# psipred/merizo_search

Hardware: AMD Instinct MI355X
Metric: queries/sec, exact 128-d cosine top-10 (recall@10 vs brute force = 1.0000) (higher is better)
Workload: dtype f32

## Files before the change

merizo_search_amd/csrc/ms_scan_pf16.h:

```cpp
#pragma once
#include "ms_scan_pf.h"

typedef _Float16 f16x8 __attribute__((ext_vector_type(8)));
constexpr uint32_t MS_PF16_MAGIC = 0x3631464du;
#define MS_PF_ERR_F16X2 5.5e-4f
#define MS_PF_ERR_F16X1 1.05e-3f

template <int KL, int NW, bool SAMPLE, bool MASK, int NQP>
__global__ __launch_bounds__(64 * NW, NW / 4) void ms_scan_pf16_kernel(const ScanParams p) {
    static_assert(NQP == 1 || NQP == 2, "query parts");
    static_assert(NW == 4 || NW == 8, "one or two waves per SIMD");
    constexpr int PPW = 16 / NW;
#ifdef MS_STAMP
    const unsigned long long tl_entry = __builtin_amdgcn_s_memrealtime();
    unsigned long long tl_setup = 0, tl_first = 0, tl_loop = 0;
#endif
    if (ms_gate_closed(p.gate, p.gate_epoch)) return;
    extern __shared__ __attribute__((aligned(16))) char smem[];
    typedef __attribute__((address_space(3))) char lds_char_t;
    typedef volatile __attribute__((address_space(3))) uint32_t lds_flag_t;
    typedef __attribute__((address_space(3))) ms_u32x2 lds_cand_t;
    const int tid = threadIdx.x, lane = tid & 63;
    const int wave = __builtin_amdgcn_readfirstlane(tid >> 6);
    const int r = lane & 31, h = lane >> 5;
    lds_flag_t *arrived = (lds_flag_t *)((lds_char_t *)smem + PF2_OFF_CNT);
    const float *auxring = reinterpret_cast<const float *>(smem + PF2_OFF_AUX);

    const int bid = blockIdx.x;
    const int per_super = 8 * p.n_qgroups;
    const int super = bid / per_super, within = bid % per_super;
    const int stream = super * 8 + (within & 7);
    const int qg = within >> 3;
    if (stream >= p.n_streams) return;
    const int64_t row_begin = (int64_t)stream * p.rows_per_stream;
    const int64_t row_end = (row_begin + p.rows_per_stream < p.n) ? row_begin + p.rows_per_stream : p.n;
    const int nfull = (int)((row_end - row_begin) >> 6);
    const int rem = (int)((row_end - row_begin) & 63);
    const int ntl = SAMPLE ? (nfull < p.max_tiles ? nfull : p.max_tiles) : nfull + (rem > 0 ? 1 : 0);
    constexpr bool mask_on = MASK;

    const int qtile = qg * NW + wave;
    const bool has_q = qtile < p.n_qtiles;
    if (tid < PF2_ARR) arrived[tid] = 0u;
    __syncthreads();
    const uint32_t ring_lds = __builtin_amdgcn_readfirstlane((uint32_t)(uintptr_t)(lds_char_t *)smem);

    const uint32_t voff = (uint32_t)(16 * lane);
    const uint64_t img0 = (uint64_t)(uintptr_t)p.pf_image + (uint64_t)(row_begin >> 6) * 16384u + (uint32_t)(1024 * PPW) * (uint32_t)wave;
    uint64_t it_sb = 0;
    uint32_t it_dst = 0;
    auto issue_prep = [&](int t) __attribute__((always_inline)) {
        const uint64_t b = img0 + (uint64_t)t * 16384u;
        const uint32_t b_lo = (uint32_t)__builtin_amdgcn_readfirstlane((uint32_t)b);
        const uint32_t b_hi = (uint32_t)__builtin_amdgcn_readfirstlane((uint32_t)(b >> 32));
        it_sb = ((uint64_t)b_hi << 32) | (uint64_t)b_lo;
        it_dst = (uint32_t)__builtin_amdgcn_readfirstlane(ring_lds + (uint32_t)(t % PF2_R) * 16384u + (uint32_t)(1024 * PPW) * (uint32_t)wave);
    };
    auto issue_piece = [&](auto i_c) __attribute__((always_inline)) {
        constexpr int I = decltype(i_c)::value;
        if constexpr (I < PPW) {
            const uint32_t d = (uint32_t)__builtin_amdgcn_readfirstlane(it_dst);
            const uint32_t lo = (uint32_t)__builtin_amdgcn_readfirstlane((uint32_t)it_sb), hi = (uint32_t)__builtin_amdgcn_readfirstlane((uint32_t)(it_sb >> 32));
            ms_glds_s16<1024 * I>(d + 1024 * I, voff, ((uint64_t)hi << 32) | (uint64_t)lo);
        }
    };
    auto issue_aux = [&](int t) __attribute__((always_inline)) {
        if constexpr (MASK) {
            int64_t row = row_begin + (int64_t)t * 64 + lane;
            if (row >= p.n) row = p.n - 1;
            const uint32_t dst = wave == 0 ? ring_lds + PF2_OFF_AUX + (uint32_t)(t % PF2_AUXR) * 256u
                                           : ring_lds + PF2_OFF_DUMMY + (uint32_t)(wave - 1) * 256u;
            ms_glds_v4((uint32_t)__builtin_amdgcn_readfirstlane(dst), p.lengths + row);
        }
    };
    auto issue_tile = [&](int t) __attribute__((always_inline)) {
        issue_prep(t);
        issue_piece(std::integral_constant<int, 0>{}); issue_piece(std::integral_constant<int, 1>{});
        issue_piece(std::integral_constant<int, 2>{}); issue_piece(std::integral_constant<int, 3>{});
        issue_aux(t);
    };
    auto wait_own = [&](auto n_c) __attribute__((always_inline)) {
        constexpr int N = decltype(n_c)::value;
        ms_pf2_vmcnt<(PPW + (MASK ? 1 : 0)) * N>();
    };
    const uint32_t arr_lds = ring_lds + PF2_OFF_CNT;
    auto publish = [&](int t) __attribute__((always_inline)) {
        const uint32_t a_ = arr_lds + 4u * (uint32_t)(t & (PF2_ARR - 1));
        uint32_t pub_a, pub_one;
        asm volatile("v_mov_b32 %0, %2\n\tv_mov_b32 %1, 1\n\ts_mov_b64 exec, 1\n\tds_add_u32 %0, %1\n\ts_mov_b64 exec, -1"
                     : "=&v"(pub_a), "=&v"(pub_one) : "s"(a_) : "memory");
    };
    uint32_t seen = 0;
    auto read_arrived = [&](int t) __attribute__((always_inline)) { seen = arrived[t & (PF2_ARR - 1)]; };
    auto wait_arrived = [&](int t) __attribute__((always_inline)) {
        const uint32_t need = (uint32_t)NW * (uint32_t)(t / PF2_ARR + 1);
        uint32_t sv_, spins_, av_;
        static_assert(PF2_ARR == 16, "the mask below");
        asm volatile("s_waitcnt lgkmcnt(0)\n\t"
                     "v_readfirstlane_b32 %0, %2\n\t"
                     "s_cmp_ge_u32 %0, %5\n\t"
                     "s_setprio 2\n\t"
                     "s_cbranch_scc1 2f\n\t"
                     "s_setprio 0\n\t"
                     "s_and_b32 %0, %4, 15\n\t"
                     "s_lshl_b32 %0, %0, 2\n\t"
                     "s_add_u32 %0, %0, %6\n\t"
                     "v_mov_b32 %3, %0\n\t"
                     "s_mov_b32 %1, 0\n\t"
                     "1:\n\t"
                     "s_sleep 1\n\t"
                     "ds_read_b32 %2, %3\n\t"
                     "s_add_u32 %1, %1, 1\n\t"
                     "s_waitcnt lgkmcnt(0)\n\t"
                     "v_readfirstlane_b32 %0, %2\n\t"
                     "s_cmp_ge_u32 %0, %5\n\t"
                     "s_cbranch_scc1 2f\n\t"
                     "s_cmp_lt_u32 %1, 0x1000000\n\t"
                     "s_cbranch_scc1 1b\n\t"
                     "s_trap 2\n\t"
                     "2:"
                     : "=&s"(sv_), "=&s"(spins_), "+v"(seen), "=&v"(av_) : "s"(t), "s"(need), "s"(arr_lds) : "memory", "scc");
        asm volatile("" ::: "memory");
    };
    const int qidx = qtile * 32 + r;
    const bool q_valid = qidx < p.nq;
    const bool hist_on = !SAMPLE && p.hist != nullptr && p.lb_s != nullptr;
    f32x4 qv[16];
    float pre_lb = -INFINITY, pre_stp = 0.0f, pre_qlen = 0.0f;
    uint32_t pre_magic = MS_PF16_MAGIC, pre_n = (uint32_t)p.n;
    int pre_sr = 0;
    if (has_q) {
        const uint32_t *trailer = reinterpret_cast<const uint32_t *>(reinterpret_cast<const char *>(p.pf_image) + (size_t)((p.n + 63) >> 6) * 16384u);
        pre_magic = trailer[0];
        pre_sr = (int)trailer[1];
        pre_n = trailer[2];
        const f32x4 *src = reinterpret_cast<const f32x4 *>(p.qn + (size_t)(q_valid ? qidx : 0) * MS_DIM + 64 * h);
#pragma unroll
        for (int i = 0; i < 16; ++i) qv[i] = src[i];
        if (!SAMPLE && p.lb_s != nullptr) pre_lb = p.lb_s[qidx];
        if (hist_on && q_valid) pre_stp = p.hstep[qidx];
        if (MASK && p.qlen != nullptr && q_valid) pre_qlen = p.qlen[qidx];
    }
    asm volatile("" ::: "memory");
#pragma unroll
    for (int t = 0; t < PF2_D; ++t)
        if (t < ntl) issue_tile(t);

    if (!has_q) {
        if (ntl > 0) {
            if (ntl >= PF2_D) wait_own(std::integral_constant<int, PF2_D - PF2_W>{}); else ms_pf2_vmcnt<0>();
#pragma unroll
            for (int t = 0; t < PF2_W; ++t)
                if (t < ntl) publish(t);
        }
        for (int t = 0; t < ntl; ++t) {
            if (t + 1 < ntl) { read_arrived(t + 1); wait_arrived(t + 1); }
            if (t + PF2_D < ntl) {
                issue_tile(t + PF2_D);
                wait_own(std::integral_constant<int, PF2_D - PF2_W>{});
            } else {
                ms_pf2_vmcnt<0>();
            }
            if (t + PF2_W < ntl) publish(t + PF2_W);
        }
        return;
    }

    ScanState<SAMPLE ? 1 : KL> st;
    ScanHist hg;
    f16x8 qh[8], ql[NQP == 2 ? 8 : 1];
#pragma unroll
    for (int j = 0; j < (SAMPLE ? 1 : KL); ++j) { st.ls[j] = -INFINITY; st.li[j] = MS_IDX_NONE; }
    st.floor = -INFINITY;
    st.tau = -INFINITY;
    if (!SAMPLE && p.lb_s != nullptr) {
        const float lb = pre_lb;
        st.floor = (lb == -INFINITY) ? -INFINITY : nextafterf(lb, -INFINITY);
        st.tau = st.floor;
    }
    if (!q_valid) { st.floor = INFINITY; st.tau = INFINITY; }
    if (!SAMPLE && (p.debug_flags & 1)) { st.floor = INFINITY; st.tau = INFINITY; }
    hg.counters = nullptr; hg.base = 0.0f; hg.step = 0.0f; hg.inv_step = 0.0f;
    if (hist_on && q_valid) {
        const float stp = pre_stp, lb = pre_lb;
        if (stp > 0.0f && lb > -INFINITY) { hg.counters = p.hist + (size_t)qidx * 16; hg.base = lb; hg.step = stp; hg.inv_step = 1.0f / stp; }
    }
    float up = 1.0f, down = 1.0f;
    {
        const uint32_t magic = (uint32_t)__builtin_amdgcn_readfirstlane((int)pre_magic);
        const int sr = __builtin_amdgcn_readfirstlane(pre_sr);
        const uint32_t img_n = (uint32_t)__builtin_amdgcn_readfirstlane((int)pre_n);
        if (magic != MS_PF16_MAGIC || img_n != (uint32_t)p.n) __builtin_trap();
        f32x4 v[16];
        float m = 0.0f;
        float rinv = 1.0f;
        if (p.qraw_eps > 0.0f) {
            float ss = 0.0f;
#pragma unroll
            for (int i = 0; i < 16; ++i) { ss += qv[i].x * qv[i].x; ss += qv[i].y * qv[i].y; ss += qv[i].z * qv[i].z; ss += qv[i].w * qv[i].w; }
            ss = ss + ms_xor32_f(ss, h);
            rinv = 1.0f / fmaxf(sqrtf(ss), p.qraw_eps);
        }
#pragma unroll
        for (int i = 0; i < 16; ++i) {
            v[i] = q_valid ? qv[i] * rinv : f32x4{0.0f, 0.0f, 0.0f, 0.0f};
            m = fmaxf(m, fmaxf(fmaxf(fabsf(v[i].x), fabsf(v[i].y)), fmaxf(fabsf(v[i].z), fabsf(v[i].w))));
        }
        m = fmaxf(m, ms_xor32_f(m, h));
        int sq = 0;
        if (m > 0.0f && m < INFINITY) sq = 13 - ((int)((__float_as_uint(m) >> 23) & 0xFFu) - 127);
        sq = sq > 60 ? 60 : (sq < -60 ? -60 : sq);
        const float qs = __uint_as_float((uint32_t)(127 + sq) << 23);
        up = __uint_as_float((uint32_t)(127 + sr + sq) << 23);
        down = __uint_as_float((uint32_t)(127 - sr - sq) << 23);
#pragma unroll
        for (int b = 0; b < 8; ++b) {
            const f32x4 a0 = v[2 * b] * qs, a1 = v[2 * b + 1] * qs;
            const float x[8] = {a0.x, a0.y, a0.z, a0.w, a1.x, a1.y, a1.z, a1.w};
#pragma unroll
            for (int j = 0; j < 8; ++j) {
                const float c = fminf(fmaxf(x[j], -65504.0f), 65504.0f);
                const _Float16 hi16 = (_Float16)c;
                qh[b][j] = hi16;
                if constexpr (NQP == 2) ql[b][j] = (_Float16)(c - (float)hi16);
            }
        }
    }
    float tau_s = st.tau * up;
    const float my_qlen = (mask_on && p.qlen != nullptr && q_valid) ? pre_qlen : 0.0f;
    const float qlen_eff = mask_on ? my_qlen : INFINITY;
    const float mincov_eff = mask_on ? p.mincov : 0.0f;
    float smax = -INFINITY;
    auto apply_mask = [&](f32x16 &acc, int t, int half) __attribute__((always_inline)) {
        const f32x4 *ax = reinterpret_cast<const f32x4 *>(auxring + (t & (PF2_AUXR - 1)) * 64 + 32 * half + 4 * h);
#pragma unroll
        for (int g = 0; g < 4; ++g) {
            const f32x4 len4 = ax[2 * g];
#pragma unroll
            for (int j = 0; j < 4; ++j) {
                const float mk = (qlen_eff >= len4[j] * mincov_eff) ? 1.0f : 0.0f;
                acc[4 * g + j] = acc[4 * g + j] * mk;
            }
        }
    };
    bool neg_tau = !SAMPLE && mask_on && (__ballot(st.tau < 0.0f) != 0);
    const bool pace_on = !SAMPLE && p.prog != nullptr;
    constexpr int PACE_LEAD = 48;
    int pace_left = 16384;
    auto pace = [&](int t) __attribute__((always_inline)) {
        if (wave != 0 || (t & 15) != 0) return;
        const uint64_t line = (uint64_t)(uintptr_t)(p.prog + (size_t)stream * 16);
        const uint32_t l_lo = (uint32_t)__builtin_amdgcn_readfirstlane((uint32_t)line), l_hi = (uint32_t)__builtin_amdgcn_readfirstlane((uint32_t)(line >> 32));
        const uint64_t sline = ((uint64_t)l_hi << 32) | (uint64_t)l_lo;
        const uint32_t tag = p.prog_epoch << 24;
        if (lane == 0) __hip_atomic_store(p.prog + (size_t)stream * 16 + qg, tag | (uint32_t)t, __ATOMIC_RELAXED, __HIP_MEMORY_SCOPE_AGENT);
        if (t < PACE_LEAD) return;
        typedef uint32_t u32x16_ __attribute__((ext_vector_type(16)));
        for (; pace_left > 0; --pace_left) {
            u32x16_ w;
            asm volatile("s_load_dwordx16 %0, %1, 0x0 glc\n\ts_waitcnt lgkmcnt(0)" : "=s"(w) : "s"(sline) : "memory");
            uint32_t mn = 0xFFFFFFu;
#pragma unroll
            for (int i = 0; i < 16; ++i) {
                const uint32_t v = ((w[i] >> 24) == p.prog_epoch) ? (w[i] & 0xFFFFFFu) : 0u;
                if (i < p.n_qgroups) mn = v < mn ? v : mn;
            }
            if ((uint32_t)t <= mn + (uint32_t)PACE_LEAD) break;
            __builtin_amdgcn_s_sleep(64);
        }
    };
    auto retau = [&]() __attribute__((always_inline)) { tau_s = st.tau * up; };

    uint32_t ccnt = 0;
    auto cand_slot = [&](uint32_t c) __attribute__((always_inline)) -> lds_cand_t * {
        return (lds_cand_t *)((lds_char_t *)smem + PF2_OFF_CAND + (wave * PF2_CAND) * 512) + c * 64 + lane;
    };
    auto flush = [&]() __attribute__((always_inline)) {
        for (uint32_t c = 0; __ballot(ccnt > c) != 0; ++c) {
            const ms_u32x2 e = *cand_slot(c < PF2_CAND ? c : 0);
            const float v = (ccnt > c) ? __uint_as_float(e.x) : -INFINITY;
            ms_lane_insert<SAMPLE ? 1 : KL>(st, v, e.y, 0, h);
            ms_lane_insert<SAMPLE ? 1 : KL>(st, v, e.y, 1, h);
        }
        ccnt = 0;
        retau();
    };
    constexpr bool VISIT2 = !(MASK && (NQP == 2 || KL >= 16));
    auto visit_v2 = [&](f32x16 &sc_v, int t, int half, bool check_rows) __attribute__((always_inline)) {
        if (mask_on) apply_mask(sc_v, t, half);
        const uint32_t sub_row0 = (uint32_t)(row_begin + (int64_t)t * 64) + (uint32_t)(32 * half + 4 * h);
#pragma unroll 1
        for (;;) {
            bool ovf = false;
            float g0, g1, g2, g3;
            asm("v_max3_f32 %0, %4, %5, %6\n\tv_max3_f32 %1, %8, %9, %10\n\tv_max3_f32 %2, %12, %13, %14\n\tv_max3_f32 %3, %16, %17, %18\n\t"
                "v_max_f32 %0, %0, %7\n\tv_max_f32 %1, %1, %11\n\tv_max_f32 %2, %2, %15\n\tv_max_f32 %3, %3, %19"
                : "=&v"(g0), "=&v"(g1), "=&v"(g2), "=&v"(g3)
                : "v"(sc_v[0]), "v"(sc_v[1]), "v"(sc_v[2]), "v"(sc_v[3]), "v"(sc_v[4]), "v"(sc_v[5]), "v"(sc_v[6]), "v"(sc_v[7]), "v"(sc_v[8]),
                  "v"(sc_v[9]), "v"(sc_v[10]), "v"(sc_v[11]), "v"(sc_v[12]), "v"(sc_v[13]), "v"(sc_v[14]), "v"(sc_v[15]));
#define MS_PF16_REG(I)                                                                                                   \
            {                                                                                                            \
                const float ss = sc_v[I];                                                                                \
                const uint32_t row = sub_row0 + (uint32_t)(8 * ((I) >> 2) + ((I) & 3));                                    \
                bool pass = ss > tau_s;                                                                                  \
                if (check_rows) pass = pass && ((int64_t)row < row_end);                                                 \
                if (pass) {                                                                                              \
                    if (ccnt < (uint32_t)PF2_CAND) {                                                                     \
                        const float s_ = ss * down;                       \
                        if (hg.counters != nullptr) ms_hist_count(hg, s_);                                               \
                        *cand_slot(ccnt) = ms_u32x2{__float_as_uint(s_), row};                                           \
                        ccnt += 1;                                                                                       \
                        sc_v[I] = -INFINITY;                                                                             \
                    } else {                                                                                             \
                        ovf = true;                                                                                      \
                    }                                                                                                    \
                }                                                                                                        \
            }
#define MS_PF16_GROUP(G, GM) if (__ballot(GM > tau_s) != 0) { MS_PF16_REG(4 * (G)) MS_PF16_REG(4 * (G) + 1) MS_PF16_REG(4 * (G) + 2) MS_PF16_REG(4 * (G) + 3) }
            MS_PF16_GROUP(0, g0) MS_PF16_GROUP(1, g1) MS_PF16_GROUP(2, g2) MS_PF16_GROUP(3, g3)
#undef MS_PF16_GROUP
#undef MS_PF16_REG
            if (__builtin_expect(__ballot(ovf) == 0, 1)) break;
            flush();
        }
    };
    auto visit_v1 = [&](f32x16 &sc_v, int t, int half, bool check_rows) __attribute__((always_inline)) {
        if (mask_on) apply_mask(sc_v, t, half);
        const uint32_t sub_row0 = (uint32_t)(row_begin + (int64_t)t * 64) + (uint32_t)(32 * half + 4 * h);
        uint32_t regs = 0;
        {
            float g0, g1, g2, g3;
            asm("v_max3_f32 %0, %4, %5, %6\n\tv_max3_f32 %1, %8, %9, %10\n\tv_max3_f32 %2, %12, %13, %14\n\tv_max3_f32 %3, %16, %17, %18\n\t"
                "v_max_f32 %0, %0, %7\n\tv_max_f32 %1, %1, %11\n\tv_max_f32 %2, %2, %15\n\tv_max_f32 %3, %3, %19"
                : "=&v"(g0), "=&v"(g1), "=&v"(g2), "=&v"(g3)
                : "v"(sc_v[0]), "v"(sc_v[1]), "v"(sc_v[2]), "v"(sc_v[3]), "v"(sc_v[4]), "v"(sc_v[5]), "v"(sc_v[6]), "v"(sc_v[7]), "v"(sc_v[8]),
                  "v"(sc_v[9]), "v"(sc_v[10]), "v"(sc_v[11]), "v"(sc_v[12]), "v"(sc_v[13]), "v"(sc_v[14]), "v"(sc_v[15]));
#define MS_PF16_GROUP(G, GM)                                                                                             \
            if (__ballot(GM > tau_s) != 0) {                                                                             \
                _Pragma("unroll") for (int j = 0; j < 4; ++j) regs |= (__ballot(sc_v[4 * (G) + j] > tau_s) != 0 ? 1u : 0u) << (4 * (G) + j); \
            }
            MS_PF16_GROUP(0, g0) MS_PF16_GROUP(1, g1) MS_PF16_GROUP(2, g2) MS_PF16_GROUP(3, g3)
#undef MS_PF16_GROUP
        }
#pragma unroll 1
        while (regs != 0u) {
            const int i = __builtin_ctz(regs);
            regs &= regs - 1u;
            const uint64_t m0_ = (i & 1) ? ~0ull : 0ull, m1_ = (i & 2) ? ~0ull : 0ull, m2_ = (i & 4) ? ~0ull : 0ull, m3_ = (i & 8) ? ~0ull : 0ull;
            float l1[8], l2[4], l3[2], ss;
#define MS_SEL(D, A, B, M) asm("v_cndmask_b32 %0, %1, %2, %3" : "=v"(D) : "v"(A), "v"(B), "s"(M))
#pragma unroll
            for (int j = 0; j < 8; ++j) MS_SEL(l1[j], sc_v[2 * j], sc_v[2 * j + 1], m0_);
#pragma unroll
            for (int j = 0; j < 4; ++j) MS_SEL(l2[j], l1[2 * j], l1[2 * j + 1], m1_);
            MS_SEL(l3[0], l2[0], l2[1], m2_); MS_SEL(l3[1], l2[2], l2[3], m2_);
            MS_SEL(ss, l3[0], l3[1], m3_);
#undef MS_SEL
            const uint32_t row = sub_row0 + (uint32_t)(8 * (i >> 2) + (i & 3));
            const float s = ss * down;
            bool pass = ss > tau_s;
            if (check_rows) pass = pass && ((int64_t)row < row_end);
            if (pass) {
                if (hg.counters != nullptr) ms_hist_count(hg, s);
                *cand_slot(ccnt) = ms_u32x2{__float_as_uint(s), row};
                ccnt += 1;
            }
            if (__builtin_expect(__ballot(ccnt >= PF2_CAND) != 0, 0)) flush();
        }
    };
    auto visit = [&](f32x16 &sc_v, int t, int half, bool check_rows) __attribute__((always_inline)) {
        if constexpr (VISIT2) visit_v2(sc_v, t, half, check_rows); else visit_v1(sc_v, t, half, check_rows);
    };

#ifdef MS_STAMP
    unsigned long long sp_t0 = 0, sp_sync = 0, sp_vis = 0, sp_nvis = 0, sp_chain = 0, sp_hist = 0, sp_lgkm = 0, sp_flow = 0;
#define PF2_T0() sp_t0 = __builtin_amdgcn_s_memtime()
#define PF2_ACC(V) { const unsigned long long now_ = __builtin_amdgcn_s_memtime(); V += now_ - sp_t0; sp_t0 = now_; }
#else
#define PF2_T0()
#define PF2_ACC(V)
#endif
    f32x4 fr[16];
    f32x16 acc0, acc1;
#pragma unroll
    for (int i = 0; i < 16; ++i) { acc0[i] = -INFINITY; acc1[i] = -INFINITY; }

    auto frag_base = [&](int t) __attribute__((always_inline)) -> const f32x4 * {
        return reinterpret_cast<const f32x4 *>(smem + (size_t)(t % PF2_R) * 16384 + 16 * lane);
    };
    auto filter = [&](int t, f32x16 &pv0, f32x16 &pv1) __attribute__((always_inline)) {
        if (SAMPLE) {
            if (mask_on && t > 0) { apply_mask(pv0, t - 1, 0); apply_mask(pv1, t - 1, 1); }
#pragma unroll
            for (int i = 0; i < 16; ++i) { smax = (pv0[i] > smax) ? pv0[i] : smax; smax = (pv1[i] > smax) ? pv1[i] : smax; }
        } else {
            float mx, mx1;
#define MS_PF16_MAX(M, PV)                                                                                                                        \
            asm("v_max3_f32 %0, %1, %2, %3\n\tv_max3_f32 %0, %0, %4, %5\n\tv_max3_f32 %0, %0, %6, %7\n\tv_max3_f32 %0, %0, %8, %9\n\t"             \
                "v_max3_f32 %0, %0, %10, %11\n\tv_max3_f32 %0, %0, %12, %13\n\tv_max3_f32 %0, %0, %14, %15\n\tv_max_f32 %0, %0, %16"               \
                : "=&v"(M) : "v"(PV[0]), "v"(PV[1]), "v"(PV[2]), "v"(PV[3]), "v"(PV[4]), "v"(PV[5]), "v"(PV[6]), "v"(PV[7]), "v"(PV[8]), "v"(PV[9]), \
                  "v"(PV[10]), "v"(PV[11]), "v"(PV[12]), "v"(PV[13]), "v"(PV[14]), "v"(PV[15]))
            MS_PF16_MAX(mx, pv0);
            MS_PF16_MAX(mx1, pv1);
#undef MS_PF16_MAX
            const bool hit0 = __ballot(mx > tau_s) != 0, hit1 = __ballot(mx1 > tau_s) != 0;
            if (__builtin_expect(hit0 || hit1 || neg_tau, 0)) {
                PF2_T0();
                if (t > 0) {
                    if (hit0 || neg_tau) visit(pv0, t - 1, 0, false);
                    if (hit1 || neg_tau) visit(pv1, t - 1, 1, false);
                }
                if (mask_on) neg_tau = __ballot(st.tau < 0.0f) != 0;
#ifdef MS_STAMP
                sp_nvis += 1;
#endif
                PF2_ACC(sp_vis)
            }
        }
    };
    auto stage = [&](auto steady_c, int t, f32x16 &out0, f32x16 &out1) __attribute__((always_inline)) {
        constexpr bool STEADY = decltype(steady_c)::value;
        PF2_T0();
        asm volatile("s_waitcnt lgkmcnt(0)" ::: "memory");
        PF2_ACC(sp_lgkm)
        if (STEADY || t + 1 < ntl) wait_arrived(t + 1);
        PF2_ACC(sp_sync)
        filter(t, out0, out1);
#pragma unroll
        for (int i = 0; i < 16; ++i) { out0[i] = 0.0f; out1[i] = 0.0f; }
        const f32x4 *src = frag_base(t + 1);
        const bool issuing = STEADY || t + PF2_D < ntl;
#define MS_PF2_BLOCK(B)                                                                                               \
        {                                                                                                             \
            const f16x8 f0 = __builtin_bit_cast(f16x8, fr[2 * (B)]), f1 = __builtin_bit_cast(f16x8, fr[2 * (B) + 1]);   \
            out0 = __builtin_amdgcn_mfma_f32_32x32x16_f16(f0, qh[B], out0, 0, 0, 0);                                  \
            out1 = __builtin_amdgcn_mfma_f32_32x32x16_f16(f1, qh[B], out1, 0, 0, 0);                                  \
            if constexpr (NQP == 2) {                                                                                 \
                out0 = __builtin_amdgcn_mfma_f32_32x32x16_f16(f0, ql[B], out0, 0, 0, 0);                              \
                out1 = __builtin_amdgcn_mfma_f32_32x32x16_f16(f1, ql[B], out1, 0, 0, 0);                              \
            }                                                                                                         \
            __builtin_amdgcn_sched_barrier(0);                                                                        \
            fr[2 * (B)] = src[64 * (2 * (B))];                                                                        \
            fr[2 * (B) + 1] = src[64 * (2 * (B) + 1)];                                                                \
        }
        MS_PF2_BLOCK(0)
        __builtin_amdgcn_sched_barrier(0);
        MS_PF2_BLOCK(1)
        if (STEADY || issuing) issue_prep(t + PF2_D);
        __builtin_amdgcn_sched_barrier(0);
        MS_PF2_BLOCK(2)
        if (STEADY || issuing) issue_piece(std::integral_constant<int, 0>{});
        __builtin_amdgcn_sched_barrier(0);
        MS_PF2_BLOCK(3)
        if (STEADY || issuing) issue_piece(std::integral_constant<int, 1>{});
        __builtin_amdgcn_sched_barrier(0);
        MS_PF2_BLOCK(4)
        if (STEADY || issuing) issue_piece(std::integral_constant<int, 2>{});
        __builtin_amdgcn_sched_barrier(0);
        MS_PF2_BLOCK(5)
        if (STEADY || issuing) { issue_piece(std::integral_constant<int, 3>{}); issue_aux(t + PF2_D); }
        __builtin_amdgcn_sched_barrier(0);
        MS_PF2_BLOCK(6)
        PF2_ACC(sp_chain)
        if (STEADY || issuing) wait_own(std::integral_constant<int, PF2_D - PF2_W>{}); else ms_pf2_vmcnt<0>();
        PF2_ACC(sp_flow)
        if (STEADY || t + PF2_W < ntl) publish(t + PF2_W);
        read_arrived(t + 2);
        __builtin_amdgcn_sched_barrier(0);
        MS_PF2_BLOCK(7)
#undef MS_PF2_BLOCK
#ifdef MS_STAMP
        asm volatile("s_nop 0" : "+v"(out0), "+v"(out1));
#endif
        PF2_ACC(sp_chain)
    };

#ifdef MS_STAMP
    const unsigned long long sp_c0 = __builtin_amdgcn_s_memtime(), sp_r0 = __builtin_amdgcn_s_memrealtime();
    tl_setup = sp_r0;
#endif
    if (ntl > 0) {
        if (ntl >= PF2_D) wait_own(std::integral_constant<int, PF2_D - PF2_W>{}); else ms_pf2_vmcnt<0>();
#pragma unroll
        for (int t = 0; t < PF2_W; ++t)
            if (t < ntl) publish(t);
        read_arrived(0);
        wait_arrived(0);
#ifdef MS_STAMP
        tl_first = __builtin_amdgcn_s_memrealtime();
#endif
        {
            const f32x4 *src = frag_base(0);
#pragma unroll
            for (int f = 0; f < 16; ++f) fr[f] = src[64 * f];
        }
        read_arrived(1);
        const int fetch_phase = 2 * wave, read_phase = (2 * wave + 2) & (HIST_PERIOD - 1);
        const int hist_area = wave & 3;
        auto hist_step = [&](int t) __attribute__((always_inline)) {
            const int phase = t & (HIST_PERIOD - 1);
            if (phase == fetch_phase) {
                const uint64_t hb = (uint64_t)(uintptr_t)p.hist + (uint64_t)qtile * 2048u;
                const uint32_t hb_lo = (uint32_t)__builtin_amdgcn_readfirstlane((uint32_t)hb);
                const uint32_t hb_hi = (uint32_t)__builtin_amdgcn_readfirstlane((uint32_t)(hb >> 32));
                const uint64_t shb = ((uint64_t)hb_hi << 32) | (uint64_t)hb_lo;
                const uint32_t dst = (uint32_t)__builtin_amdgcn_readfirstlane(ring_lds + PF2_OFF_HIST + (uint32_t)hist_area * 2048u);
                ms_glds_s16_sc1<0>(dst, voff, shb);
                ms_glds_s16_sc1<1024>(dst + 1024, voff, shb);
            }
            if (phase == read_phase && t >= 2) {
                PF2_T0();
                if (t - 1 + PF2_D < ntl) wait_own(std::integral_constant<int, 2>{}); else ms_pf2_vmcnt<0>();
                const ms_u32x4 *hp = reinterpret_cast<const ms_u32x4 *>(smem + PF2_OFF_HIST + hist_area * 2048 + r * 64);
                const ms_u32x4 c0 = hp[0], c1 = hp[1], c2 = hp[2], c3 = hp[3];
                const uint32_t c[16] = {c0.x, c0.y, c0.z, c0.w, c1.x, c1.y, c1.z, c1.w, c2.x, c2.y, c2.z, c2.w, c3.x, c3.y, c3.z, c3.w};
                uint32_t cum = 0;
                int n_lt = 0;
#pragma unroll
                for (int j = 15; j >= 0; --j) { cum += c[j]; n_lt += (cum < (uint32_t)p.k) ? 1 : 0; }
                const int J = 15 - n_lt;
                if (hg.counters != nullptr && J >= 1) {
                    st.floor = fmaxf(st.floor, ms_next_below(ms_hist_edge(hg, J)));
                    st.tau = fmaxf(st.tau, st.floor);
                }
                asm volatile("s_waitcnt lgkmcnt(0)" ::: "memory");
                retau();
                if (mask_on) neg_tau = __ballot(st.tau < 0.0f) != 0;
                PF2_ACC(sp_hist)
            }
        };
        int t = 0;
        for (; t + PF2_D < ntl; ++t) {
            if ((t & 1) == 0) {
                if (pace_on) pace(t);
                if (hist_on) hist_step(t);
            }
            stage(std::true_type{}, t, acc0, acc1);
        }
        for (; t < ntl; ++t) {
            if ((t & 1) == 0 && hist_on) hist_step(t);
            stage(std::false_type{}, t, acc0, acc1);
        }
#ifdef MS_STAMP
        if (!SAMPLE && lane == 0 && p.stamps != nullptr && (size_t)bid * 64 + 64 <= 4 * 4 * 65536) {
            unsigned long long *o = p.stamps + ((size_t)bid * 8 + wave) * 8;
            tl_loop = __builtin_amdgcn_s_memrealtime();
            o[0] = __builtin_amdgcn_s_memtime() - sp_c0;
            o[1] = __builtin_amdgcn_s_memrealtime() - sp_r0;
            o[2] = (unsigned long long)ntl;
            o[3] = (sp_lgkm << 32) | (sp_flow & 0xFFFFFFFFull);
            o[4] = sp_vis; o[5] = sp_nvis; o[6] = sp_chain; o[7] = (sp_hist << 32) | (sp_sync & 0xFFFFFFFFull);
        }
#endif
        if (pace_on && wave == 0 && lane == 0)
            __hip_atomic_store(p.prog + (size_t)stream * 16 + qg, (p.prog_epoch << 24) | 0xFFFFFFu, __ATOMIC_RELAXED, __HIP_MEMORY_SCOPE_AGENT);
        if (SAMPLE) {
            if (mask_on) { apply_mask(acc0, ntl - 1, 0); apply_mask(acc1, ntl - 1, 1); }
#pragma unroll
            for (int i = 0; i < 16; ++i) { smax = (acc0[i] > smax) ? acc0[i] : smax; smax = (acc1[i] > smax) ? acc1[i] : smax; }
        } else {
            visit(acc0, ntl - 1, 0, true);
            visit(acc1, ntl - 1, 1, true);
            flush();
        }
    }

    if (SAMPLE) {
        smax = smax * down;
        const float other = ms_xor32_f(smax, h);
        if (h == 0) {
            const float hi = (other > smax) ? other : smax, lo = (other > smax) ? smax : other;
            const size_t o = ((size_t)stream * p.nq_pad + qidx) * p.k;
            p.part_s[o] = hi;
            p.part_i[o] = (hi > -INFINITY) ? (uint32_t)(2 * stream) : MS_IDX_NONE;
            if (p.k > 1) {
                p.part_s[o + 1] = lo;
                p.part_i[o + 1] = (lo > -INFINITY) ? (uint32_t)(2 * stream + 1) : MS_IDX_NONE;
            }
        }
        return;
    }
#pragma unroll
    for (int j = 0; j < (SAMPLE ? 1 : KL); ++j) {
        const int rank = h * KL + j;
        if (rank < p.k) {
            const size_t o = ((size_t)stream * p.nq_pad + qidx) * p.k + rank;
            p.part_s[o] = st.ls[j];
            p.part_i[o] = st.li[j];
        }
    }
#ifdef MS_STAMP
    if (!SAMPLE && lane == 0 && p.stamps != nullptr && bid < 4096) {
        asm volatile("s_waitcnt vmcnt(0)" ::: "memory");
        unsigned long long *o = p.stamps + 8 * 8 * 4096 + ((size_t)bid * 8 + wave) * 8;
        o[0] = tl_entry; o[1] = tl_setup; o[2] = tl_first; o[3] = tl_loop; o[4] = __builtin_amdgcn_s_memrealtime();
    }
#endif
}

template <int KL, int NW, bool MASK, int NQP>
int launch_scan_pf16(const ScanPlan &pl, const ScanParams &sp, hipStream_t st) {
    MS_HIP_CHECK(hipFuncSetAttribute(reinterpret_cast<const void *>(ms_scan_pf16_kernel<KL, NW, false, MASK, NQP>),
                                     hipFuncAttributeMaxDynamicSharedMemorySize, (int)PF2_LDS));
    hipLaunchKernelGGL((ms_scan_pf16_kernel<KL, NW, false, MASK, NQP>), dim3(pl.d.grid), dim3(64 * NW), PF2_LDS, st, sp);
    MS_LAUNCH_CHECK("ms_scan_pf16_kernel");
    return MS_OK;
}
template <int KL, int NW>
int launch_scan_pf16_any(const ScanPlan &pl, const ScanParams &sp, hipStream_t st) {
    const bool two = sp.pf_format == MS_PF_F16X2;
    if (sp.lengths != nullptr) return two ? launch_scan_pf16<KL, NW, true, 2>(pl, sp, st) : launch_scan_pf16<KL, NW, true, 1>(pl, sp, st);
    return two ? launch_scan_pf16<KL, NW, false, 2>(pl, sp, st) : launch_scan_pf16<KL, NW, false, 1>(pl, sp, st);
}

int ms_launch_scan_pf16_kl5(const ScanPlan &pl, const ScanParams &sp, hipStream_t st);
int ms_launch_scan_pf16_kl10(const ScanPlan &pl, const ScanParams &sp, hipStream_t st);
int ms_launch_scan_pf16_kl16(const ScanPlan &pl, const ScanParams &sp, hipStream_t st);
int ms_launch_scan_pf16_kl32(const ScanPlan &pl, const ScanParams &sp, hipStream_t st);
int ms_launch_sample_pf16(const ScanPlan &pl, const ScanParams &sp, hipStream_t st);
int ms_launch_pf16_build_image(const float *db, int64_t n, int sr, void *image, hipStream_t st);
```

merizo_search_amd/csrc/ms_scan_pf16_kl5.hip:

```cpp
#include "ms_scan_pf16.h"

int ms_launch_scan_pf16_kl5(const ScanPlan &pl, const ScanParams &sp, hipStream_t st) {
    return sp.qpw == 2 ? launch_scan_pf16_any<5, 8>(pl, sp, st) : launch_scan_pf16_any<5, 4>(pl, sp, st);
}

template <int NW, bool MASK, int NQP>
static int launch_sample_pf16(const ScanPlan &pl, const ScanParams &sp, hipStream_t st) {
    MS_HIP_CHECK(hipFuncSetAttribute(reinterpret_cast<const void *>(ms_scan_pf16_kernel<5, NW, true, MASK, NQP>),
                                     hipFuncAttributeMaxDynamicSharedMemorySize, (int)PF2_LDS));
    hipLaunchKernelGGL((ms_scan_pf16_kernel<5, NW, true, MASK, NQP>), dim3(pl.d.grid), dim3(64 * NW), PF2_LDS, st, sp);
    MS_LAUNCH_CHECK("ms_scan_pf16_kernel (sample)");
    return MS_OK;
}
template <int NW>
static int launch_sample_pf16_any(const ScanPlan &pl, const ScanParams &sp, hipStream_t st) {
    const bool two = sp.pf_format == MS_PF_F16X2;
    if (sp.lengths != nullptr) return two ? launch_sample_pf16<NW, true, 2>(pl, sp, st) : launch_sample_pf16<NW, true, 1>(pl, sp, st);
    return two ? launch_sample_pf16<NW, false, 2>(pl, sp, st) : launch_sample_pf16<NW, false, 1>(pl, sp, st);
}

int ms_launch_sample_pf16(const ScanPlan &pl, const ScanParams &sp, hipStream_t st) {
    return sp.qpw == 2 ? launch_sample_pf16_any<8>(pl, sp, st) : launch_sample_pf16_any<4>(pl, sp, st);
}

__global__ __launch_bounds__(256) void ms_pf16_build_image_kernel(const float *db, int64_t n, char *image, int64_t ntiles, int sr) {
    const int lane = threadIdx.x & 63, r = lane & 31, h = lane >> 5;
    const float scale = __uint_as_float((uint32_t)(127 + sr) << 23);
    for (int64_t U = (int64_t)blockIdx.x * 4 + (threadIdx.x >> 6); U < 2 * ntiles; U += (int64_t)gridDim.x * 4) {
        const int64_t T = U >> 1;
        const int half = (int)(U & 1);
        const int64_t row = T * 64 + 32 * half + r;
        f32x4 x[16];
#pragma unroll
        for (int t = 0; t < 16; ++t) {
            x[t] = f32x4{0.0f, 0.0f, 0.0f, 0.0f};
            if (row < n) x[t] = *reinterpret_cast<const f32x4 *>(db + row * MS_DIM + 64 * h + 4 * t);
        }
        char *dst = image + T * 16384 + 16 * lane;
#pragma unroll
        for (int b = 0; b < 8; ++b) {
            const f32x4 a0 = x[2 * b] * scale, a1 = x[2 * b + 1] * scale;
            const float v[8] = {a0.x, a0.y, a0.z, a0.w, a1.x, a1.y, a1.z, a1.w};
            f16x8 o;
#pragma unroll
            for (int j = 0; j < 8; ++j) {
                o[j] = (_Float16)fminf(fmaxf(v[j], -65504.0f), 65504.0f);
            }
            *reinterpret_cast<f16x8 *>(dst + 1024 * (2 * b + half)) = o;
        }
    }
    if (blockIdx.x == 0 && threadIdx.x < 64) {
        uint32_t *tr = reinterpret_cast<uint32_t *>(image + ntiles * 16384);
        uint32_t w = 0u;
        if (threadIdx.x == 0) w = MS_PF16_MAGIC;
        if (threadIdx.x == 1) w = (uint32_t)sr;
        if (threadIdx.x == 2) w = (uint32_t)(n & 0xFFFFFFFFll);
        if (threadIdx.x == 3) w = (uint32_t)(n >> 32);
        tr[threadIdx.x] = w;
    }
}

int ms_launch_pf16_build_image(const float *db, int64_t n, int sr, void *image, hipStream_t st) {
    const int64_t ntiles = (n + 63) / 64;
    int64_t blocks = (2 * ntiles + 3) / 4;
    if (blocks < 1) blocks = 1;
    hipLaunchKernelGGL(ms_pf16_build_image_kernel, dim3((unsigned)(blocks < 16384 ? blocks : 16384)), dim3(256), 0, st, db, n, (char *)image, ntiles, sr);
    MS_LAUNCH_CHECK("ms_pf16_build_image_kernel");
    return MS_OK;
}
```

Baseline: 485,600.

## Stage query loads through LDS, coalesce partial top-k writes, and trim kernel prologue

Query vectors are now fetched with direct global-to-LDS loads into the ring slot and then read back into registers with an XOR swizzle, replacing strided per-lane global loads. Only wave 0 reads the image trailer and passes the shift factor through an extra LDS word, and the early barrier is merged into a single later one. The per-query partial top-k results are staged in LDS and written out as contiguous coalesced stores, and the final tile uses the cheaper filter path when there is no remainder. The change also adds fine-grained timeline stamps under MS_STAMP, uses 64 extra bytes of LDS, and makes the prologue synchronisation harder to verify.

New measurement: 484,900. About the same (-0.1%).

```diff
diff --git a/merizo_search_amd/csrc/ms_scan_pf16.h b/merizo_search_amd/csrc/ms_scan_pf16.h
--- a/merizo_search_amd/csrc/ms_scan_pf16.h
+++ b/merizo_search_amd/csrc/ms_scan_pf16.h
@@ -2,6 +2,9 @@
 #include "ms_scan_pf.h"
 
 typedef _Float16 f16x8 __attribute__((ext_vector_type(8)));
+constexpr int PF16_OFF_SR = PF2_LDS;
+constexpr int PF16_LDS = PF2_LDS + 64;
+static_assert(PF16_LDS <= 160 * 1024, "LDS of one CU");
 constexpr uint32_t MS_PF16_MAGIC = 0x3631464du;
 #define MS_PF_ERR_F16X2 5.5e-4f
 #define MS_PF_ERR_F16X1 1.05e-3f
@@ -14,8 +17,13 @@
 #ifdef MS_STAMP
     const unsigned long long tl_entry = __builtin_amdgcn_s_memrealtime();
     unsigned long long tl_setup = 0, tl_first = 0, tl_loop = 0;
+    unsigned tl_fine[11] = {0u, 0u, 0u, 0u, 0u, 0u, 0u, 0u, 0u, 0u, 0u};
+#define PF16_FINE(I) { asm volatile("" ::: "memory"); tl_fine[I] = (unsigned)(__builtin_amdgcn_s_memrealtime() - tl_entry); asm volatile("" ::: "memory"); }
+#else
+#define PF16_FINE(I)
 #endif
     if (ms_gate_closed(p.gate, p.gate_epoch)) return;
+    PF16_FINE(0)
     extern __shared__ __attribute__((aligned(16))) char smem[];
     typedef __attribute__((address_space(3))) char lds_char_t;
     typedef volatile __attribute__((address_space(3))) uint32_t lds_flag_t;
@@ -42,7 +50,6 @@
     const int qtile = qg * NW + wave;
     const bool has_q = qtile < p.n_qtiles;
     if (tid < PF2_ARR) arrived[tid] = 0u;
-    __syncthreads();
     const uint32_t ring_lds = __builtin_amdgcn_readfirstlane((uint32_t)(uintptr_t)(lds_char_t *)smem);
 
     const uint32_t voff = (uint32_t)(16 * lane);
@@ -127,24 +134,52 @@
     const bool hist_on = !SAMPLE && p.hist != nullptr && p.lb_s != nullptr;
     f32x4 qv[16];
     float pre_lb = -INFINITY, pre_stp = 0.0f, pre_qlen = 0.0f;
-    uint32_t pre_magic = MS_PF16_MAGIC, pre_n = (uint32_t)p.n;
-    int pre_sr = 0;
+    volatile __attribute__((address_space(3))) int *sr_word = (volatile __attribute__((address_space(3))) int *)((lds_char_t *)smem + PF16_OFF_SR);
     if (has_q) {
-        const uint32_t *trailer = reinterpret_cast<const uint32_t *>(reinterpret_cast<const char *>(p.pf_image) + (size_t)((p.n + 63) >> 6) * 16384u);
-        pre_magic = trailer[0];
-        pre_sr = (int)trailer[1];
-        pre_n = trailer[2];
-        const f32x4 *src = reinterpret_cast<const f32x4 *>(p.qn + (size_t)(q_valid ? qidx : 0) * MS_DIM + 64 * h);
-#pragma unroll
-        for (int i = 0; i < 16; ++i) qv[i] = src[i];
+        {
+            const uint64_t qb = (uint64_t)(uintptr_t)p.qn;
+            const uint32_t qb_lo = (uint32_t)__builtin_amdgcn_readfirstlane((uint32_t)qb), qb_hi = (uint32_t)__builtin_amdgcn_readfirstlane((uint32_t)(qb >> 32));
+            const uint64_t sqb = ((uint64_t)qb_hi << 32) | (uint64_t)qb_lo;
+            const uint32_t qslot = (uint32_t)__builtin_amdgcn_readfirstlane(ring_lds + 16384u * (uint32_t)wave);
+#pragma unroll
+            for (int s = 0; s < 16; ++s) {
+                const int g = lane ^ (s & 7);
+                const int qs = qtile * 32 + 2 * s + (g >> 5);
+                const uint32_t off = (uint32_t)(qs < p.nq ? qs : 0) * (uint32_t)(MS_DIM * 4) + 16u * (uint32_t)(g & 31);
+                ms_glds_s16<0>(qslot + 1024u * (uint32_t)s, off, sqb);
+            }
+        }
+        ms_u32x4 tr = ms_u32x4{MS_PF16_MAGIC, 0u, (uint32_t)p.n, 0u};
+        if (wave == 0)
+            tr = *reinterpret_cast<const ms_u32x4 *>(reinterpret_cast<const char *>(p.pf_image) + (size_t)((p.n + 63) >> 6) * 16384u);
         if (!SAMPLE && p.lb_s != nullptr) pre_lb = p.lb_s[qidx];
         if (hist_on && q_valid) pre_stp = p.hstep[qidx];
         if (MASK && p.qlen != nullptr && q_valid) pre_qlen = p.qlen[qidx];
+        PF16_FINE(1)
+        asm volatile("s_waitcnt vmcnt(0)" ::: "memory");
+        {
+            const int s = r >> 1, x = s & 7;
+            const f32x4 *src = reinterpret_cast<const f32x4 *>(smem + (size_t)wave * 16384 + 16 * (64 * s + 32 * (r & 1) + 16 * h));
+#pragma unroll
+            for (int i = 0; i < 16; ++i) qv[i] = src[i ^ x];
+        }
+        if (wave == 0) {
+            const uint32_t magic = (uint32_t)__builtin_amdgcn_readfirstlane((int)tr.x);
+            const uint32_t img_n = (uint32_t)__builtin_amdgcn_readfirstlane((int)tr.z);
+            if (magic != MS_PF16_MAGIC || img_n != (uint32_t)p.n) __builtin_trap();
+            if (lane == 0) *sr_word = (int)tr.y;
+        }
+#pragma unroll
+        for (int i = 0; i < 16; ++i) asm volatile("" : "+v"(qv[i]));
+        asm volatile("s_waitcnt lgkmcnt(0)" : "+v"(pre_lb), "+v"(pre_stp), "+v"(pre_qlen) : : "memory");
+        PF16_FINE(2)
     }
-    asm volatile("" ::: "memory");
+    __syncthreads();
+    PF16_FINE(3)
 #pragma unroll
     for (int t = 0; t < PF2_D; ++t)
         if (t < ntl) issue_tile(t);
+    PF16_FINE(4)
 
     if (!has_q) {
         if (ntl > 0) {
@@ -187,10 +222,9 @@
     }
     float up = 1.0f, down = 1.0f;
     {
-        const uint32_t magic = (uint32_t)__builtin_amdgcn_readfirstlane((int)pre_magic);
-        const int sr = __builtin_amdgcn_readfirstlane(pre_sr);
-        const uint32_t img_n = (uint32_t)__builtin_amdgcn_readfirstlane((int)pre_n);
-        if (magic != MS_PF16_MAGIC || img_n != (uint32_t)p.n) __builtin_trap();
+        const int sr = __builtin_amdgcn_readfirstlane(*sr_word);
+#pragma unroll
+        for (int i = 0; i < 16; ++i) asm volatile("" : "+v"(qv[i]));
         f32x4 v[16];
         float m = 0.0f;
         float rinv = 1.0f;
@@ -201,6 +235,10 @@
             ss = ss + ms_xor32_f(ss, h);
             rinv = 1.0f / fmaxf(sqrtf(ss), p.qraw_eps);
         }
+#ifdef MS_STAMP
+        asm volatile("" : "+v"(rinv));
+        PF16_FINE(6)
+#endif
 #pragma unroll
         for (int i = 0; i < 16; ++i) {
             v[i] = q_valid ? qv[i] * rinv : f32x4{0.0f, 0.0f, 0.0f, 0.0f};
@@ -225,6 +263,11 @@
                 if constexpr (NQP == 2) ql[b][j] = (_Float16)(c - (float)hi16);
             }
         }
+#ifdef MS_STAMP
+#pragma unroll
+        for (int b = 0; b < 8; ++b) { asm volatile("" : "+v"(qh[b])); if constexpr (NQP == 2) asm volatile("" : "+v"(ql[b])); }
+        PF16_FINE(7)
+#endif
     }
     float tau_s = st.tau * up;
     const float my_qlen = (mask_on && p.qlen != nullptr && q_valid) ? pre_qlen : 0.0f;
@@ -484,6 +527,7 @@
 #pragma unroll
         for (int t = 0; t < PF2_W; ++t)
             if (t < ntl) publish(t);
+        PF16_FINE(8)
         read_arrived(0);
         wait_arrived(0);
 #ifdef MS_STAMP
@@ -542,9 +586,9 @@
             stage(std::false_type{}, t, acc0, acc1);
         }
 #ifdef MS_STAMP
+        tl_loop = __builtin_amdgcn_s_memrealtime();
         if (!SAMPLE && lane == 0 && p.stamps != nullptr && (size_t)bid * 64 + 64 <= 4 * 4 * 65536) {
             unsigned long long *o = p.stamps + ((size_t)bid * 8 + wave) * 8;
-            tl_loop = __builtin_amdgcn_s_memrealtime();
             o[0] = __builtin_amdgcn_s_memtime() - sp_c0;
             o[1] = __builtin_amdgcn_s_memrealtime() - sp_r0;
             o[2] = (unsigned long long)ntl;
@@ -559,11 +603,30 @@
 #pragma unroll
             for (int i = 0; i < 16; ++i) { smax = (acc0[i] > smax) ? acc0[i] : smax; smax = (acc1[i] > smax) ? acc1[i] : smax; }
         } else {
-            visit(acc0, ntl - 1, 0, true);
-            visit(acc1, ntl - 1, 1, true);
+            if (rem > 0) {
+                visit(acc0, ntl - 1, 0, true);
+                visit(acc1, ntl - 1, 1, true);
+            } else {
+                filter(ntl, acc0, acc1);
+            }
+            PF16_FINE(9)
             flush();
+            PF16_FINE(10)
         }
     }
+#ifdef MS_STAMP
+    auto write_timeline = [&]() __attribute__((always_inline)) {
+        if (lane == 0 && p.stamps != nullptr && bid < 4096) {
+            asm volatile("s_waitcnt vmcnt(0)" ::: "memory");
+            unsigned long long *o = p.stamps + 8 * 8 * 4096 + ((size_t)bid * 8 + wave) * 8;
+            auto f16 = [&](int i) -> unsigned long long { return (unsigned long long)(tl_fine[i] < 65535u ? tl_fine[i] : 65535u); };
+            o[0] = tl_entry; o[1] = tl_setup; o[2] = tl_first; o[3] = tl_loop; o[4] = __builtin_amdgcn_s_memrealtime();
+            o[5] = f16(0) | (f16(1) << 16) | (f16(2) << 32) | (f16(3) << 48);
+            o[6] = f16(4) | (f16(5) << 16) | (f16(6) << 32) | (f16(7) << 48);
+            o[7] = f16(8) | (f16(9) << 16) | (f16(10) << 32) | ((unsigned long long)(SAMPLE ? 2 : 1) << 48);
+        }
+    };
+#endif
 
     if (SAMPLE) {
         smax = smax * down;
@@ -578,31 +641,47 @@
                 p.part_i[o + 1] = (lo > -INFINITY) ? (uint32_t)(2 * stream + 1) : MS_IDX_NONE;
             }
         }
+#ifdef MS_STAMP
+        write_timeline();
+#endif
         return;
     }
-#pragma unroll
-    for (int j = 0; j < (SAMPLE ? 1 : KL); ++j) {
-        const int rank = h * KL + j;
-        if (rank < p.k) {
-            const size_t o = ((size_t)stream * p.nq_pad + qidx) * p.k + rank;
-            p.part_s[o] = st.ls[j];
-            p.part_i[o] = st.li[j];
+    if constexpr (!SAMPLE) {
+        const int kk = p.k;
+        int qr = 32;
+        while (qr * kk > PF2_CAND * 128) qr >>= 1;
+        typedef __attribute__((address_space(3))) uint32_t lds_u32_t;
+        lds_u32_t *stg = (lds_u32_t *)((lds_char_t *)smem + PF2_OFF_CAND + (wave * PF2_CAND) * 512);
+        const size_t o0 = ((size_t)stream * p.nq_pad + (size_t)qtile * 32) * kk;
+        uint32_t *out_s = reinterpret_cast<uint32_t *>(p.part_s) + o0, *out_i = p.part_i + o0;
+        for (int r0 = 0; r0 < 32; r0 += qr) {
+            const bool mine = r >= r0 && r < r0 + qr;
+            const int base = (r - r0) * kk + h * KL;
+            const int cnt = qr * kk;
+            if (mine) {
+#pragma unroll
+                for (int j = 0; j < KL; ++j)
+                    if (h * KL + j < kk) stg[base + j] = __float_as_uint(st.ls[j]);
+            }
+            for (int e = lane; e < cnt; e += 64) out_s[r0 * kk + e] = stg[e];
+            if (mine) {
+#pragma unroll
+                for (int j = 0; j < KL; ++j)
+                    if (h * KL + j < kk) stg[base + j] = st.li[j];
+            }
+            for (int e = lane; e < cnt; e += 64) out_i[r0 * kk + e] = stg[e];
         }
     }
 #ifdef MS_STAMP
-    if (!SAMPLE && lane == 0 && p.stamps != nullptr && bid < 4096) {
-        asm volatile("s_waitcnt vmcnt(0)" ::: "memory");
-        unsigned long long *o = p.stamps + 8 * 8 * 4096 + ((size_t)bid * 8 + wave) * 8;
-        o[0] = tl_entry; o[1] = tl_setup; o[2] = tl_first; o[3] = tl_loop; o[4] = __builtin_amdgcn_s_memrealtime();
-    }
+    write_timeline();
 #endif
 }
 
 template <int KL, int NW, bool MASK, int NQP>
 int launch_scan_pf16(const ScanPlan &pl, const ScanParams &sp, hipStream_t st) {
     MS_HIP_CHECK(hipFuncSetAttribute(reinterpret_cast<const void *>(ms_scan_pf16_kernel<KL, NW, false, MASK, NQP>),
-                                     hipFuncAttributeMaxDynamicSharedMemorySize, (int)PF2_LDS));
-    hipLaunchKernelGGL((ms_scan_pf16_kernel<KL, NW, false, MASK, NQP>), dim3(pl.d.grid), dim3(64 * NW), PF2_LDS, st, sp);
+                                     hipFuncAttributeMaxDynamicSharedMemorySize, (int)PF16_LDS));
+    hipLaunchKernelGGL((ms_scan_pf16_kernel<KL, NW, false, MASK, NQP>), dim3(pl.d.grid), dim3(64 * NW), PF16_LDS, st, sp);
     MS_LAUNCH_CHECK("ms_scan_pf16_kernel");
     return MS_OK;
 }
diff --git a/merizo_search_amd/csrc/ms_scan_pf16_kl5.hip b/merizo_search_amd/csrc/ms_scan_pf16_kl5.hip
--- a/merizo_search_amd/csrc/ms_scan_pf16_kl5.hip
+++ b/merizo_search_amd/csrc/ms_scan_pf16_kl5.hip
@@ -7,8 +7,8 @@
 template <int NW, bool MASK, int NQP>
 static int launch_sample_pf16(const ScanPlan &pl, const ScanParams &sp, hipStream_t st) {
     MS_HIP_CHECK(hipFuncSetAttribute(reinterpret_cast<const void *>(ms_scan_pf16_kernel<5, NW, true, MASK, NQP>),
-                                     hipFuncAttributeMaxDynamicSharedMemorySize, (int)PF2_LDS));
-    hipLaunchKernelGGL((ms_scan_pf16_kernel<5, NW, true, MASK, NQP>), dim3(pl.d.grid), dim3(64 * NW), PF2_LDS, st, sp);
+                                     hipFuncAttributeMaxDynamicSharedMemorySize, (int)PF16_LDS));
+    hipLaunchKernelGGL((ms_scan_pf16_kernel<5, NW, true, MASK, NQP>), dim3(pl.d.grid), dim3(64 * NW), PF16_LDS, st, sp);
     MS_LAUNCH_CHECK("ms_scan_pf16_kernel (sample)");
     return MS_OK;
 }
```
